# hsientzucheng/CP-360-Weakly-Supervised-Saliency

Hardware: AMD Instinct MI355X
Metric: frames/sec end-to-end 1024x2048 equi->saliency (higher is better)
Workload: dtype bf16+f16; 1 GPU; C3/C4 per-GPU shard: 4 clips x 16 frames 1024x2048 u8 equi -> 6x224^2 cube -> CubePad ResNet-50 -> CAM -> ConvLSTM x16 -> cube_to_equi saliency 14x28; clips_per_gpu=4, frames_per_clip=16, cube_dim=224, graph_replay=False, temporal_stage_dtype=bf16, static_stage_dtype=f16, static_stage_fp16_fallback=False, parallelism=clips sharded over 1 GPU(s), 1 all-gather of maps, pipelining=SaliencyEngine.stream: two HIP streams, fill + drain inside the timed region

## Files before the change

### cp_360_weakly_supervised_saliency_amd/csrc/conv_igemm.hip

```cpp
#include "common.h"
#include <stdio.h>
#include <stdlib.h>

#include "conv_common.h"

template <typename T, int MJ>
__device__ __forceinline__ void epilogue_direct(const ConvK& p, f32x4 (&acc)[4][MJ], int n0, int m0, int wch0, int wrow0,
                                                int lane, int rows_valid) {
    constexpr int JB = sizeof(T) == 4 ? 2 : 5;
    const int ml = lane & 15;
    const T* res = reinterpret_cast<const T*>(p.res);
    T* outp = reinterpret_cast<T*>(p.out);
    const int rlim = min(rows_valid, p.M - m0);
#pragma unroll
    for (int pr = 0; pr < 2; ++pr) {
        const int n = n0 + wch0 + pr * 32 + (lane >> 4) * 8;
        const bool nok = n < p.c_out;
        float bb[8] = {0.f, 0.f, 0.f, 0.f, 0.f, 0.f, 0.f, 0.f};
        if (p.bias && nok) {
            const float4 t0 = *reinterpret_cast<const float4*>(p.bias + n);
            const float4 t1 = *reinterpret_cast<const float4*>(p.bias + n + 4);
            bb[0] = t0.x; bb[1] = t0.y; bb[2] = t0.z; bb[3] = t0.w; bb[4] = t1.x; bb[5] = t1.y; bb[6] = t1.z; bb[7] = t1.w;
        }
#pragma unroll
// ... 765 lines not shown
#undef CP360_RING_TAIL
    }

    const int ml = lane & 15;
    if (!p.partial && p.epi_direct) {
        epilogue_direct<T, MJ>(p, acc, n0, m0, wch0, wrow0, lane, BM);
        return;
    }
    if (!p.partial && (p.c_out % EPC == 0) && (p.ld_out % EPC == 0) && (p.out_coff % EPC == 0) &&
        (p.ld_res % EPC == 0)) {
        epilogue_lds<T, BN, BM, MJ, 512, G::template lds_bytes<T>()>(p, lds, acc, n0, m0, wch0, wrow0, lane, tid);
        return;
    }
#pragma unroll
    for (int i = 0; i < 4; ++i) {
        const int n = n0 + wch0 + acc_chan(i, lane);
        if (n >= p.c_out) continue;
#pragma unroll
        for (int j = 0; j < MJ; ++j) {
            const int m = m0 + wrow0 + j * 16 + ml;
            if (m >= p.M) continue;
            float v[4] = {acc[i][j][0], acc[i][j][1], acc[i][j][2], acc[i][j][3]};
            if (p.partial) {
                store4(p.partial + ((size_t)split * p.M + m) * p.c_out + (p.slab_rows ? slab_col(n) : n), v);
            } else {
                if (p.bias) {
                    const float4 bb = *reinterpret_cast<const float4*>(p.bias + n);
                    v[0] += bb.x; v[1] += bb.y; v[2] += bb.z; v[3] += bb.w;
                }
                if (p.res) {
                    float r[4];
                    load4(reinterpret_cast<const T*>(p.res) + (size_t)m * p.ld_res + n, r);
                    v[0] += r[0]; v[1] += r[1]; v[2] += r[2]; v[3] += r[3];
                }
                if (p.relu) {
                    v[0] = fmaxf(v[0], 0.f); v[1] = fmaxf(v[1], 0.f);
                    v[2] = fmaxf(v[2], 0.f); v[3] = fmaxf(v[3], 0.f);
                }
                store4(reinterpret_cast<T*>(p.out) + (size_t)m * p.ld_out + p.out_coff + n, v);
            }
        }
    }
}

template <typename T, int BM>
__global__ __launch_bounds__(512, 2) void conv_igemm_ring_kernel(const ConvK p) {
    typedef RingGeom<BM> G;
    __shared__ __attribute__((aligned(1024))) unsigned char lds[G::template lds_bytes<T>()];

    const int tid = threadIdx.x, lane = tid & 63;
    const int wave = __builtin_amdgcn_readfirstlane(tid >> 6);
    int n0, m0, split;
    {
        const int nwg = p.nt * p.mt * p.splits;
        const int L = blockIdx.x, xcd = L & 7, q = nwg >> 3, r = nwg & 7;
        int w = (xcd < r ? xcd * (q + 1) : r * (q + 1) + (xcd - r) * q) + (L >> 3);
        if (p.reverse) w = nwg - 1 - w;
        int nt_i, mt_i;
        if (p.m_fast) {
            mt_i = w % p.mt;
            const int rest = w / p.mt;
            nt_i = rest % p.nt;
            split = rest / p.nt;
        } else {
            nt_i = w % p.nt;
            const int rest = w / p.nt;
            mt_i = rest % p.mt;
            split = rest / p.mt;
        }
        n0 = nt_i * G::BN;
        m0 = mt_i * BM;
    }
    if constexpr (BM == 256) {
        if (wave < 4) ring_body<T, 256, 8, 4, false>(p, lds, n0, m0, split, wave, lane, tid, (wave >> 1) * 64, (wave & 1) * 128);
        else          ring_body<T, 256, 8, 4, true>(p, lds, n0, m0, split, wave, lane, tid, (wave >> 1) * 64, (wave & 1) * 128);
    } else if constexpr (BM == 160) {
        if (wave < 4) ring_body<T, 160, 5, 3, false>(p, lds, n0, m0, split, wave, lane, tid, (wave >> 1) * 64, (wave & 1) * 80);
        else          ring_body<T, 160, 5, 3, true>(p, lds, n0, m0, split, wave, lane, tid, (wave >> 1) * 64, (wave & 1) * 80);
    } else {
        static_assert(BM == 304, "pixel tile is 160, 256 or 304");
        if (wave < 4) ring_body<T, 304, 10, 5, false>(p, lds, n0, m0, split, wave, lane, tid, wave * 64, 0);
        else          ring_body<T, 304, 9, 5, true>(p, lds, n0, m0, split, wave, lane, tid, (wave - 4) * 64, 160);
    }
}

template <typename T>
__global__ __launch_bounds__(512, 4) void conv_igemm_ring2_kernel(const ConvK p) {
    typedef RingGeom<128, 2> G;
    __shared__ __attribute__((aligned(1024))) unsigned char lds[G::template lds_bytes<T>()];
    const int tid = threadIdx.x, lane = tid & 63;
    const int wave = __builtin_amdgcn_readfirstlane(tid >> 6);
    int n0, m0, split;
    {
        const int nwg = p.nt * p.mt * p.splits;
        const int L = blockIdx.x, xcd = L & 7, q = nwg >> 3, r = nwg & 7;
        int w = (xcd < r ? xcd * (q + 1) : r * (q + 1) + (xcd - r) * q) + (L >> 3);
        if (p.reverse) w = nwg - 1 - w;
        int nt_i, mt_i;
        if (p.m_fast) {
            mt_i = w % p.mt;
            const int rest = w / p.mt;
            nt_i = rest % p.nt;
            split = rest / p.nt;
        } else {
            nt_i = w % p.nt;
            const int rest = w / p.nt;
            mt_i = rest % p.mt;
            split = rest / p.mt;
        }
        n0 = nt_i * G::BN;
        m0 = mt_i * 128;
    }
    if (wave < 4) ring_body<T, 128, 4, 2, false, 2>(p, lds, n0, m0, split, wave, lane, tid, (wave >> 1) * 64, (wave & 1) * 64);
    else          ring_body<T, 128, 4, 2, true, 2>(p, lds, n0, m0, split, wave, lane, tid, (wave >> 1) * 64, (wave & 1) * 64);
}

__device__ __forceinline__ int clip_swz(int row) { return ((row >> 2) & 1) << 1; }

template <int MODE> struct ClipGeom {
    static constexpr bool FACE = MODE == 1, HALF = MODE == 2;
    static constexpr int BN = 256, BM = FACE ? 256 : HALF ? 192 : 304, NW = 6, NA = 2;
    static constexpr int RROWS = FACE ? 336 : HALF ? 384 : 304;
    static constexpr int GROUP_ROWS = FACE ? 128 : HALF ? 96 : 160;
    static constexpr int XW = (RROWS - 256) / 16;
    static constexpr int WSTAGE = BN * 64;
    static constexpr int ATILE = RROWS * 64;
    static constexpr int TAB_ROW = 32;
    static constexpr int TAB_BYTES = 9 * 2 * 16 * TAB_ROW;
    static constexpr int OFF_ACT = NW * WSTAGE;
    static constexpr int OFF_TAB = OFF_ACT + NA * ATILE;
    static constexpr int LDS_BYTES = OFF_TAB + TAB_BYTES;
};

template <typename T, int MJ, int JH, bool LAG, int MODE>
__device__ __forceinline__ void clip_body(const ConvK& p, unsigned char* lds, const int n0, const int clip, const int split,
                                          const int wave, const int lane, const int tid, const int wch0, const int grp) {
    typedef ClipGeom<MODE> G;
    constexpr bool FACE = G::FACE, HALF = G::HALF;
    constexpr int BN = G::BN, BM = G::BM;
    constexpr int EPC = Elem<T>::EPC;
    constexpr int BKS = 4 * EPC;
    constexpr int TAPS = 9;
    const int wrow0 = grp * G::GROUP_ROWS;
    const bool xw = wave < G::XW;
    const int rows_valid = FACE ? 256 : HALF ? 192 : p.clip_rows;
    const int m0 = clip * rows_valid;

    const int drow = 16 * wave + (lane >> 2);
    const int dchunk = (lane & 3) ^ ((0 - ((4 * wave + (lane >> 4)) & 3)) & 3);
    const int dchunk_a = (lane & 3) ^ clip_swz(drow);
    const T* in = reinterpret_cast<const T*>(p.in);
    const T* wbase = reinterpret_cast<const T*>(p.w) + (size_t)(n0 / 256) * 256 * p.k_total + drow * BKS + dchunk * EPC;
    constexpr int wpass = 128 * BKS;
    constexpr int WSTEP = 256 * BKS;
    const unsigned lds_base = (unsigned)(size_t)lds;
    const unsigned lds_wave = lds_base + (unsigned)(16 * wave) * 64;
    int aoff[3];
#pragma unroll
    for (int q = 0; q < 3; ++q) {
        const int r = drow + 128 * q;
        int off = -1;
        if (FACE) {
            if (r < 18 * 18 && (q < 2 || xw)) {
                const int cube = clip / 6, f = clip - cube * 6;
                const CubePadGeom geom{16, 1, 1, 1, 1};
                off = (cube * 6 * 256 + cubepad_src(f, r / 18, r - (r / 18) * 18, geom)) * p.pix_stride;
// ... 388 lines not shown
__global__ __launch_bounds__(256) void pack_weights_kernel(const float* __restrict__ w, const float* __restrict__ scale,
                                                           T* __restrict__ packed, int c_out, int c_out_pad, int c_in,
                                                           int c_pad, int kh, int kw, int stem_mode, int chan_major,
                                                           const float* __restrict__ w2, const float* __restrict__ scale2,
                                                           int c_in2, int c_pad2) {
    const int taps = kh * kw;
    constexpr int BKS = 64 / (int)sizeof(T);
    const int ktot = taps * c_pad + c_pad2;
    const long long total = (long long)c_out_pad * ktot;
    for (long long idx = (long long)blockIdx.x * blockDim.x + threadIdx.x; idx < total;
         idx += (long long)gridDim.x * blockDim.x) {
        int c, tap, n;
        if (c_pad2 > 0) {
            const int k = (int)(idx % ktot);
            n = (int)(idx / ktot);
            tap = min(k / c_pad, taps);
            c = k - tap * c_pad;
        } else if (chan_major) {
            const int e = (int)(idx % BKS);
            long long t = idx / BKS;
            const int r = (int)(t % 256);
            t /= 256;
            tap = (int)(t % taps);
            t /= taps;
            const int cpb = c_pad / BKS;
            c = (int)(t % cpb) * BKS + e;
            n = (int)(t / cpb) * 256 + r;
        } else {
            c = (int)(idx % c_pad);
            const long long t = idx / c_pad;
            tap = (int)(t % taps);
            n = (int)(t / taps);
        }
        n = (n & ~31) + ((n >> 2) & 3) * 8 + ((n >> 4) & 1) * 4 + (n & 3);
        float v = 0.f;
        if (n < c_out && tap >= taps) {
            if (c < c_in2) v = w2[(size_t)n * c_in2 + c] * (scale2 ? scale2[n] : 1.f);
        } else if (n < c_out) {
            if (stem_mode) {
                const int kx = c >> 2, ch = c & 3, ky = tap;
                if (c < c_in && kx < 7 && ch < 3) v = w[(((size_t)n * 3 + ch) * 7 + ky) * 7 + kx];
            } else if (c < c_in) {
                const int ky = tap / kw, kx = tap - ky * kw;
                v = w[(((size_t)n * c_in + c) * kh + ky) * kw + kx];
            }
            if (scale) v *= scale[n];
        }
        if constexpr (sizeof(T) == 4)
            packed[idx] = v;
        else if constexpr (__is_same(T, f16_raw))
            packed[idx] = (f16_raw)v;
        else
            packed[idx] = f32_to_bf16(v);
    }
}

static int elem_bytes(int dtype) { return dtype == CP360_F32 ? 4 : ((dtype == CP360_BF16 || dtype == CP360_F16) ? 2 : 0); }
static int bk_of(int dtype) { return 128 / elem_bytes(dtype); }
static int c_pad_of(const cp360_conv_desc* d) {
    const int unit = d->clip_resident ? bk_of(d->dtype) / 2 : bk_of(d->dtype);
    return (d->c_in + unit - 1) / unit * unit;
}
static int round_up(int a, int b) { return (a + b - 1) / b * b; }
static int c_pad2_of(const cp360_conv_desc* d) { return d->c_in2 > 0 ? round_up(d->c_in2, bk_of(d->dtype)) : 0; }

static int small_shape_status(const cp360_conv_desc* d) {
    if (d->clip_resident || d->c_out % 8 != 0) return CP360_ERR_UNSUPPORTED;
    if (d->kh * d->kw + (d->c_in2 > 0 ? 1 : 0) > CP360_SMALL_MAX_TAPS) return CP360_ERR_UNSUPPORTED;
    const long long es = elem_bytes(d->dtype);
    if ((long long)d->n_img * d->h_in * d->w_in * d->pix_stride * es >= (1LL << 32)) return CP360_ERR_UNSUPPORTED;
    if (d->c_in2 > 0 && (long long)d->n_img * d->h_in2 * d->w_in2 * d->pix_stride2 * es >= (1LL << 32)) return CP360_ERR_UNSUPPORTED;
    if (64LL * ((long long)d->kh * d->kw * c_pad_of(d) + c_pad2_of(d)) * es >= (1LL << 32)) return CP360_ERR_UNSUPPORTED;
    if (d->dtype != CP360_F32 && (d->ld_out % 8 != 0 || d->out_coff % 8 != 0 || d->ld_res % 8 != 0)) return CP360_ERR_ALIGN;
    return CP360_OK;
}

static int check_desc(const cp360_conv_desc* d) {
    if (!d) return CP360_ERR_NULL;
    if (d->dtype != CP360_F32 && d->dtype != CP360_BF16 && d->dtype != CP360_F16) return CP360_ERR_BAD_DTYPE;
    if (d->n_img <= 0 || d->h_in <= 0 || d->w_in <= 0 || d->c_in <= 0 || d->kh <= 0 || d->kw <= 0 || d->sy <= 0 ||
        d->sx <= 0 || d->h_out <= 0 || d->w_out <= 0 || d->c_out <= 0 || d->splits < 1 || d->pix_stride <= 0)
        return CP360_ERR_BAD_SHAPE;
    const int epc = 16 / elem_bytes(d->dtype);
    if (d->tile_px != 0 && d->tile_px != 64 && d->tile_px != 128 && d->tile_px != 129 && d->tile_px != 160 && d->tile_px != 256 &&
        d->tile_px != 304 && d->tile_px != 6464)
        return CP360_ERR_BAD_SHAPE;
    if (d->tile_px == 160 && d->dtype == CP360_F32) return CP360_ERR_UNSUPPORTED;
    if (d->tile_px == 6464) {
        const int rc = small_shape_status(d);
        if (rc) return rc;
    }
    if (d->tile_px == 129 && d->dtype == CP360_F32) return CP360_ERR_UNSUPPORTED;
    if (d->slab_rows != 0 && d->slab_rows != 1) return CP360_ERR_BAD_SHAPE;
    if (d->slab_rows && d->c_out % 32 != 0) return CP360_ERR_ALIGN;
    if (d->clip_resident != 0 && d->clip_resident != 1) return CP360_ERR_BAD_SHAPE;
    if (d->clip_resident && !(d->pad_mode == 1 && d->pad == 1 && d->kh == 3 && d->kw == 3 && d->sy == 1 && d->sx == 1 &&
                              d->h_in == d->w_in && (6 * d->h_in * d->w_in <= 304 || d->h_in == 16 || d->h_in == 8) && d->c_out >= 256 &&
                              d->pix_stride >= d->c_in && d->tile_px == 0))
        return CP360_ERR_UNSUPPORTED;
    if (d->c_in2 < 0) return CP360_ERR_BAD_SHAPE;
    if (d->c_in2 > 0) {
        if (d->clip_resident || d->c_out < 256 || d->pix_stride < d->c_in) return CP360_ERR_UNSUPPORTED;
        if (d->c_in2 % epc != 0) return CP360_ERR_ALIGN;
        if (d->pix_stride2 < d->c_in2 || d->h_in2 <= 0 || d->w_in2 <= 0 || d->sy2 <= 0 || d->sx2 <= 0 ||
            (d->h_out - 1) * d->sy2 >= d->h_in2 || (d->w_out - 1) * d->sx2 >= d->w_in2)
            return CP360_ERR_BAD_SHAPE;
        if ((long long)d->n_img * d->h_in2 * d->w_in2 * d->pix_stride2 >= (1LL << 31)) return CP360_ERR_BAD_SHAPE;
    }
    if (d->c_in % epc != 0 || d->c_out % 4 != 0 || d->ld_out % 4 != 0 || d->out_coff % 4 != 0 || d->ld_res % 4 != 0)
        return CP360_ERR_ALIGN;
    if (d->ld_out < d->c_out + d->out_coff) return CP360_ERR_BAD_SHAPE;
    if (d->pad_mode) {
        if (d->n_img % 6 != 0) return CP360_ERR_BATCH_NOT_6N;
        if (d->h_in != d->w_in) return CP360_ERR_NOT_SQUARE;
        if (d->pad < 0 || d->pad > d->h_in) return CP360_ERR_BAD_SHAPE;
    }
    const int pad2 = d->pad_mode ? 2 * d->pad : 0;
    if ((d->h_out - 1) * d->sy + d->kh > d->h_in + pad2) return CP360_ERR_BAD_SHAPE;
    const int span = d->pix_stride >= d->c_in ? 1 : (d->c_in + d->pix_stride - 1) / d->pix_stride;
    if (span > 1 && d->pad_mode) return CP360_ERR_UNSUPPORTED;
    if ((d->w_out - 1) * d->sx + (d->kw - 1) + span > d->w_in + pad2) return CP360_ERR_BAD_SHAPE;
    if ((long long)d->n_img * d->h_in * d->w_in * d->pix_stride >= (1LL << 31)) return CP360_ERR_BAD_SHAPE;
    return CP360_OK;
}

extern "C" size_t cp360_conv_packed_bytes(const cp360_conv_desc* d) {
    if (check_desc(d)) return 0;
    return (size_t)round_up(d->c_out, 256) * ((size_t)d->kh * d->kw * c_pad_of(d) + c_pad2_of(d)) * elem_bytes(d->dtype);
}

extern "C" size_t cp360_conv_partial_bytes(const cp360_conv_desc* d) {
    if (check_desc(d) || d->splits <= 1) return 0;
    return (size_t)d->splits * d->n_img * d->h_out * d->w_out * d->c_out * sizeof(float);
}

struct ConvPlan {
    int bn, bm, slots, splits;
    double cost;
    long long wgs = 0;
};

static ConvPlan plan_candidate(const cp360_conv_desc* d, int bn, int bm, int slots, double t_step) {
    const long long M = (long long)d->n_img * d->h_out * d->w_out;
    const long long wgs = ((d->c_out + bn - 1) / bn) * ((M + bm - 1) / bm);
    const int bk = bk_of(d->dtype);
    const int nsteps = d->kh * d->kw * (round_up(d->c_in, bk) / bk) + c_pad2_of(d) / bk;
    if (d->dtype == CP360_F32) t_step *= 3.0;
    const double t_fixed = 4.0;
    ConvPlan best{bn, bm, slots, 1, 0.0};
    for (int s = 1; s <= 32; ++s) {
        if (s > 1 && nsteps / s < 8) break;
        const long long rounds = (wgs * s + slots - 1) / slots;
        const int steps = (nsteps + s - 1) / s;
        double cost = (double)rounds * (t_fixed + steps * t_step);
        if (s > 1) cost += 4.0 + (double)s * (double)M * d->c_out * 8.0 / 4.0e6;
        if (s == 1 || cost < best.cost) {
            best.splits = s;
            best.cost = cost;
            best.wgs = wgs * s;
        }
    }
    return best;
}

static bool small_eligible(const cp360_conv_desc* d) {
    return d->dtype == CP360_F32 && small_shape_status(d) == CP360_OK;
}

static ConvPlan plan_small(const cp360_conv_desc* d) {
    const long long M = (long long)d->n_img * d->h_out * d->w_out;
    const long long tiles = ((d->c_out + 63) / 64) * ((M + 63) / 64);
    const int bk = bk_of(d->dtype);
    const int nsteps = d->kh * d->kw * (round_up(d->c_in, bk) / bk) + c_pad2_of(d) / bk;
    const double t_step = d->dtype == CP360_F32 ? 0.7 : 0.35;
    ConvPlan best{64, 64, 1024, 1, 0.0};
    for (int s = 1; s <= 32; ++s) {
        if (s > 1 && nsteps / s < 4) break;
        const long long W = tiles * s;
        const int steps = (nsteps + s - 1) / s;
        const long long per_cu = d->dtype == CP360_F32 ? (W + 255) / 256 : (W + 1023) / 1024;
        double cost = (double)((W + 1023) / 1024) * 3.0 + (double)per_cu * steps * t_step;
        if (s > 1) cost += 4.0 + (double)s * (double)M * d->c_out * 8.0 / 4.0e6;
        if (s == 1 || cost < best.cost) {
            best.splits = s;
            best.cost = cost;
            best.wgs = W;
        }
    }
    return best;
}

static ConvPlan plan_big(const cp360_conv_desc* d);
static int clip_tiles(const cp360_conv_desc* d) { return d->h_in == 16 ? d->n_img : d->h_in == 8 ? d->n_img / 3 : d->n_img / 6; }

static ConvPlan plan_of(const cp360_conv_desc* d) {
    ConvPlan best = plan_big(d);
    if (d->tile_px == 6464) return plan_small(d);
    if (d->tile_px == 0 && small_eligible(d)) {
        const ConvPlan sm = plan_small(d);
        if (sm.cost < best.cost || best.wgs < 256) best = sm;
    }
    return best;
}

static ConvPlan plan_big(const cp360_conv_desc* d) {
    if (d->clip_resident) {
        const int wgs = ((d->c_out + 255) / 256) * clip_tiles(d);
        const int nsub = 9 * (c_pad_of(d) / (bk_of(d->dtype) / 2));
        const double t_sub = (d->dtype == CP360_F32 ? 2.7 : 0.9) * (d->h_in == 8 ? 0.7 : 1.0);
        const long long M = (long long)d->n_img * d->h_out * d->w_out;
        ConvPlan best{256, 304, 256, 1, 0.0};
        for (int s = 1; s <= 32; ++s) {
            if (s > 1 && nsub / s < 16) break;
            const int rounds = (wgs * s + 255) / 256;
            double cost = (double)rounds * (4.0 + (double)((nsub + s - 1) / s) * t_sub);
            if (s > 1) cost += 4.0 + (double)s * (double)M * d->c_out * 8.0 / 4.0e6;
            if (s == 1 || cost < best.cost) {
                best.splits = s;
                best.cost = cost;
                best.wgs = (long long)wgs * s;
            }
        }
        return best;
    }
    if (d->c_out <= 64) return plan_candidate(d, 64, 256, 512, 1.5);
    if (d->c_out < 256) return plan_candidate(d, 128, 128, 512, 1.5);
    ConvPlan best = plan_candidate(d, 256, 256, 256, 2.2);
    const ConvPlan b = plan_candidate(d, 256, 128, 256, 1.25);
    if (b.cost < best.cost) best = b;
    const ConvPlan c = plan_candidate(d, 256, 304, 256, 2.2 * 304.0 / 256.0);
    if (c.cost < best.cost) best = c;
    if (d->dtype != CP360_F32 && d->c_in2 == 0) {
        const ConvPlan t160 = plan_candidate(d, 256, 160, 256, 2.2 * 176.0 / 256.0);
        if (t160.cost < best.cost) best = t160;
    }
    const int kbytes = (d->c_in + d->c_in2) * elem_bytes(d->dtype);
    if (d->dtype != CP360_F32 && d->kh * d->kw == 1 && kbytes >= 256 && kbytes <= 512) {
        ConvPlan r2 = plan_candidate(d, 256, 128, 512, 1.25);
        r2.bm = 129;
        if (r2.cost < best.cost) best = r2;
    }
    if (d->c_in2 > 0 && best.bm == 128) best.bm = d->dtype == CP360_F32 ? 256 : 129;
    return best;
}

static void tile_of(const cp360_conv_desc* d, int* bn, int* bm, int* slots) {
    ConvPlan pl = plan_of(d);
    *bn = pl.bn;
    *bm = pl.bm;
    *slots = pl.slots;
    if (pl.bm == 64) return;
    if (d->c_out >= 256 && d->tile_px == 64) {
        *bn = 128;
        *bm = 128;
        *slots = 512;
    } else if (d->c_out >= 256 && d->tile_px) {
        *bn = 256;
        *bm = d->tile_px;
        *slots = 256;
    }
}

extern "C" int cp360_conv_suggest_splits(const cp360_conv_desc* d) {
    cp360_conv_desc t = *d;
    t.splits = 1;
    if (check_desc(&t)) return 1;
    return plan_of(&t).splits;
}

extern "C" int cp360_conv_prefer_clip(const cp360_conv_desc* d) {
    if (!d) return 0;
    cp360_conv_desc c = *d;
    c.splits = 1;
    c.tile_px = 0;
    c.clip_resident = 1;
    if (check_desc(&c)) return 0;
    cp360_conv_desc t = c;
    t.clip_resident = 0;
    if (check_desc(&t) || !small_eligible(&t)) return 1;
    return plan_big(&c).cost <= plan_small(&t).cost ? 1 : 0;
}

extern "C" int cp360_conv_plan_describe(const cp360_conv_desc* d, char* buf, size_t cap) {
    if (!d || !buf || cap == 0) return CP360_ERR_NULL;
    cp360_conv_desc t = *d;
    t.splits = 1;
    int rc = check_desc(&t);
    if (rc) return rc;
    const ConvPlan pl = plan_of(&t);
    int bn = 0, bm = 0, slots = 0;
    tile_of(&t, &bn, &bm, &slots);
    const long long M = (long long)t.n_img * t.h_out * t.w_out;
    const char* name;
    long long wgs;
    if (t.clip_resident) {
        name = t.h_in == 16 ? "conv_clip 256 ch x one 16x16 face (activations LDS-resident)"
               : t.h_in == 8 ? "conv_clip 256 ch x half a cube of 8x8 faces (the cube LDS-resident)"
                             : "conv_clip 256 ch x one cube (activations LDS-resident)";
        wgs = (long long)((t.c_out + 255) / 256) * clip_tiles(&t);
    } else if (bm == 64) {
        name = "conv_small 64 ch x 64 px (8 waves)";
        wgs = (long long)((t.c_out + 63) / 64) * ((M + 63) / 64);
    } else if (t.c_out < 256 || bn != 256) {
        const bool narrow = t.c_out <= 64;
        name = narrow ? "conv_igemm 64 ch x 256 px (4 waves)" : "conv_igemm 128 ch x 128 px (4 waves)";
        wgs = narrow ? (long long)((t.c_out + 63) / 64) * ((M + 255) / 256) : (long long)((t.c_out + 127) / 128) * ((M + 127) / 128);
    } else {
        const int px = bm == 129 ? 128 : bm;
        name = bm == 129 ? "conv_igemm_ring2 256 ch x 128 px (two workgroups per CU)"
               : bm == 304 ? "conv_igemm_ring 256 ch x 304 px" : bm == 160 ? "conv_igemm_ring 256 ch x 160 px" : bm >= 256 ? "conv_igemm_ring 256 ch x 256 px" : "conv_igemm_dma 256 ch x 128 px";
        wgs = (long long)((t.c_out + 255) / 256) * ((M + px - 1) / px);
    }
    const int n = snprintf(buf, cap, "%s, %lld workgroups x split-K %d%s, model %.0f us", name, wgs * pl.splits, pl.splits,
                           t.c_in2 > 0 ? " (+ second source)" : "", pl.cost);
    return n < 0 ? CP360_ERR_BAD_SHAPE : (n >= (int)cap ? (int)cap - 1 : n);
}

static int pack_weights_impl(const cp360_conv_desc* d, const float* w_oihw, const float* scale, const float* w2,
                             const float* scale2, void* packed, int stem_mode, void* stream);

extern "C" int cp360_conv_pack_weights(const cp360_conv_desc* d, const float* w_oihw, const float* scale, void* packed,
                                       int stem_mode, void* stream) {
    if (d && d->c_in2 > 0) return CP360_ERR_NULL;
    return pack_weights_impl(d, w_oihw, scale, nullptr, nullptr, packed, stem_mode, stream);
}

extern "C" int cp360_conv_pack_weights2(const cp360_conv_desc* d, const float* w_oihw, const float* scale,
                                        const float* w2_oi, const float* scale2, void* packed, void* stream) {
    if (!d || d->c_in2 <= 0) return CP360_ERR_BAD_SHAPE;
    if (!w2_oi) return CP360_ERR_NULL;
    return pack_weights_impl(d, w_oihw, scale, w2_oi, scale2, packed, 0, stream);
}

static int pack_weights_impl(const cp360_conv_desc* d, const float* w_oihw, const float* scale, const float* w2,
                             const float* scale2, void* packed, int stem_mode, void* stream) {
    int rc = check_desc(d);
    if (rc) return rc;
    if (!w_oihw || !packed) return CP360_ERR_NULL;
    if (stem_mode && !(d->kh == 7 && d->kw == 1 && d->c_in == 32)) return CP360_ERR_UNSUPPORTED;
    if (stem_mode && d->clip_resident) return CP360_ERR_UNSUPPORTED;
    const int c_pad = c_pad_of(d);
    const int c_out_pad = round_up(d->c_out, 256);
    const int c_pad2 = c_pad2_of(d);
    const long long total = (long long)c_out_pad * ((long long)d->kh * d->kw * c_pad + c_pad2);
    long long blocks = (total + 255) / 256;
    if (blocks > 4096) blocks = 4096;
    hipStream_t st = (hipStream_t)stream;
    if (d->dtype == CP360_F32)
        hipLaunchKernelGGL((pack_weights_kernel<float>), dim3((unsigned)blocks), dim3(256), 0, st, w_oihw, scale,
                           (float*)packed, d->c_out, c_out_pad, d->c_in, c_pad, d->kh, d->kw, stem_mode, d->clip_resident,
                           w2, scale2, d->c_in2, c_pad2);
    else if (d->dtype == CP360_F16)
        hipLaunchKernelGGL((pack_weights_kernel<f16_raw>), dim3((unsigned)blocks), dim3(256), 0, st, w_oihw, scale,
                           (f16_raw*)packed, d->c_out, c_out_pad, d->c_in, c_pad, d->kh, d->kw, stem_mode, d->clip_resident,
                           w2, scale2, d->c_in2, c_pad2);
    else
        hipLaunchKernelGGL((pack_weights_kernel<bf16_raw>), dim3((unsigned)blocks), dim3(256), 0, st, w_oihw, scale,
                           (bf16_raw*)packed, d->c_out, c_out_pad, d->c_in, c_pad, d->kh, d->kw, stem_mode, d->clip_resident,
                           w2, scale2, d->c_in2, c_pad2);
    CP360_CHECK_HIP();
    return CP360_OK;
}

template <typename T, int WN, int WM>
static void launch_conv(ConvK& k, hipStream_t st) {
    k.nt = (k.c_out + WN * 64 - 1) / (WN * 64);
    k.mt = (k.M + WM * 64 - 1) / (WM * 64);
    k.m_fast = ((long long)k.c_out * k.k_total > (long long)k.M * k.kh * k.kw * k.c_in) ? 1 : 0;
    dim3 grid((unsigned)(k.nt * k.mt * k.splits), 1, 1);
    hipLaunchKernelGGL((conv_igemm_kernel<T, WN, WM>), grid, dim3(256), 0, st, k);
}

template <typename T>
static int launch_wide(const ConvK& k, int bm, dim3 grid, hipStream_t st) {
    if (bm == 304) hipLaunchKernelGGL((conv_igemm_ring_kernel<T, 304>), grid, dim3(512), 0, st, k);
    else if (bm == 160) {
        if constexpr (sizeof(T) == 2) hipLaunchKernelGGL((conv_igemm_ring_kernel<T, 160>), grid, dim3(512), 0, st, k);
        else return CP360_ERR_UNSUPPORTED;
    } else if (bm >= 256) hipLaunchKernelGGL((conv_igemm_ring_kernel<T, 256>), grid, dim3(512), 0, st, k);
    else hipLaunchKernelGGL((conv_igemm_dma_kernel<T, 4>), grid, dim3(512), 0, st, k);
    return CP360_OK;
}

extern "C" int cp360_conv_forward(const cp360_conv_desc* d, const void* in, const void* packed_w, const float* bias,
                                  const void* residual, void* out, float* partial, void* stream) {
    return cp360_conv_forward2(d, in, nullptr, packed_w, bias, residual, out, partial, stream);
}

extern "C" int cp360_conv_forward2(const cp360_conv_desc* d, const void* in, const void* in2, const void* packed_w,
                                   const float* bias, const void* residual, void* out, float* partial, void* stream) {
    int rc = check_desc(d);
    if (rc) return rc;
    if (!in || !packed_w) return CP360_ERR_NULL;
    if ((d->c_in2 > 0) != (in2 != nullptr)) return CP360_ERR_NULL;
    if (d->splits > 1 && !partial) return CP360_ERR_NULL;
    if (d->splits == 1 && !out && !partial) return CP360_ERR_NULL;
    if (residual && d->ld_res < d->c_out) return CP360_ERR_BAD_SHAPE;
    ConvK k;
    k.in = (const unsigned char*)in;
    k.w = (const unsigned char*)packed_w;
    k.out = (unsigned char*)out;
    k.bias = bias;
    k.res = (const unsigned char*)residual;
    k.partial = (d->splits > 1 || !out) ? partial : nullptr;
    k.n_img = d->n_img; k.h_in = d->h_in; k.w_in = d->w_in; k.c_in = d->c_in; k.pix_stride = d->pix_stride;
    k.kh = d->kh; k.kw = d->kw; k.sy = d->sy; k.sx = d->sx; k.h_out = d->h_out; k.w_out = d->w_out;
    k.c_out = d->c_out; k.pad_mode = d->pad_mode; k.pad = d->pad; k.ld_out = d->ld_out; k.out_coff = d->out_coff;
    k.ld_res = d->ld_res; k.relu = d->relu; k.splits = d->splits;
    k.hw_out = d->h_out * d->w_out;
    k.M = d->n_img * k.hw_out;
    const int bk = bk_of(d->dtype);
    k.c_pad = c_pad_of(d);
    k.steps_per_tap = k.c_pad / bk;
    k.in2 = (const unsigned char*)in2;
    k.c_in2 = d->c_in2; k.c_pad2 = c_pad2_of(d); k.pix_stride2 = d->pix_stride2; k.h_in2 = d->h_in2; k.w_in2 = d->w_in2;
    k.sy2 = d->sy2; k.sx2 = d->sx2;
    k.ntap = d->kh * d->kw;
    k.nsteps = d->kh * d->kw * k.steps_per_tap + k.c_pad2 / bk;
    k.steps_per_split = (k.nsteps + d->splits - 1) / d->splits;
    k.k_total = d->kh * d->kw * k.c_pad + k.c_pad2;
    k.slab_rows = d->slab_rows;
    k.reverse = cp360_launch_reverse();
    k.clip_rows = 6 * d->h_out * d->w_out;
    k.nsub = k.k_total / (bk / 2);
    k.sub_per_split = (k.nsub + d->splits - 1) / d->splits;
    {
        const size_t wbytes = (size_t)((d->c_out + 255) / 256) * 256 * k.k_total * (d->dtype == CP360_F32 ? 4 : 2);
        k.w_pin = wbytes >= ((size_t)96 << 20) ? 8 : 0x7fffffff;
    }
    k.epi_direct = 0;
    hipStream_t st = (hipStream_t)stream;
    if (d->clip_resident) {
        const int mode = d->h_in == 16 ? 1 : d->h_in == 8 ? 2 : 0;
        k.nt = (k.c_out + 255) / 256;
        k.mt = clip_tiles(d);
        k.m_fast = 1;
        dim3 grid((unsigned)(k.nt * k.mt * k.splits), 1, 1);
#define CP360_CLIP(TT)                                                                                    \
        {                                                                                                     \
            if (mode == 1)      hipLaunchKernelGGL((conv_clip_kernel<TT, 1>), grid, dim3(512), 0, st, k);     \
            else if (mode == 2) hipLaunchKernelGGL((conv_clip_kernel<TT, 2>), grid, dim3(512), 0, st, k);     \
            else                hipLaunchKernelGGL((conv_clip_kernel<TT, 0>), grid, dim3(512), 0, st, k);     \
        }
        if (d->dtype == CP360_F32) CP360_CLIP(float)
        else if (d->dtype == CP360_F16) CP360_CLIP(f16_raw)
        else CP360_CLIP(bf16_raw)
#undef CP360_CLIP
        CP360_CHECK_HIP();
        return CP360_OK;
    }
    const bool narrow = d->c_out <= 64;
    int bn_ = 0, bm_ = 0, slots_ = 0;
    tile_of(d, &bn_, &bm_, &slots_);
    if (bm_ == 64) {
        cp360_launch_conv_small(k, d->dtype, st);
        CP360_CHECK_HIP();
        return CP360_OK;
    }
    if (d->dtype != CP360_F32 && d->kh == 1 && d->kw == 1 && d->sy == 1 && d->sx == 1 && d->pad == 0 && d->c_in == 64 &&
        d->c_out == 64 && d->c_in2 == 0 && d->splits <= 1 && !residual && d->tile_px == 0 && d->pix_stride % 8 == 0 &&
        d->ld_out % 8 == 0 && d->out_coff % 8 == 0 && k.M >= 4096 && k.out != nullptr && k.partial == nullptr) {
        long long blocks = ((long long)(k.M + 15) / 16 + 7) / 8;
        if (blocks > 256 * 8) blocks = 256 * 8;
        if (d->dtype == CP360_F16) hipLaunchKernelGGL((conv_pw64_kernel<f16_raw>), dim3((unsigned)blocks), dim3(256), 0, st, k);
        else hipLaunchKernelGGL((conv_pw64_kernel<bf16_raw>), dim3((unsigned)blocks), dim3(256), 0, st, k);
        CP360_CHECK_HIP();
        return CP360_OK;
    }
    if (d->c_out < 256) bn_ = bm_ = slots_ = 0;
    const bool wide = d->c_out >= 256 && bn_ == 256;
    if (d->c_in2 > 0) {
        if (!wide) return CP360_ERR_UNSUPPORTED;
        if (bm_ == 128) bm_ = d->dtype == CP360_F32 ? 256 : 129;
    }
    if (wide) {
        const bool big = bm_ >= 256;
        const int bm = bm_ == 129 ? 128 : bm_;
        if (bm_ == 129) k.epi_direct = d->c_out % 8 == 0 && d->ld_out % 8 == 0 && d->out_coff % 8 == 0 && d->ld_res % 8 == 0;
        k.nt = (k.c_out + 255) / 256;
        k.mt = (k.M + bm - 1) / bm;
        k.m_fast = ((long long)k.c_out * k.k_total > (long long)k.M * k.kh * k.kw * k.c_in) ? 1 : 0;
        dim3 grid((unsigned)(k.nt * k.mt * k.splits), 1, 1);
        if (d->c_in2 > 0 && !big && bm_ != 129) return CP360_ERR_UNSUPPORTED;
        if (bm_ == 129 && d->dtype == CP360_F16) hipLaunchKernelGGL((conv_igemm_ring2_kernel<f16_raw>), grid, dim3(512), 0, st, k);
        else if (bm_ == 129) hipLaunchKernelGGL((conv_igemm_ring2_kernel<bf16_raw>), grid, dim3(512), 0, st, k);
        else if (d->dtype == CP360_F32) rc = launch_wide<float>(k, bm, grid, st);
        else if (d->dtype == CP360_F16) rc = launch_wide<f16_raw>(k, bm, grid, st);
        else rc = launch_wide<bf16_raw>(k, bm, grid, st);
        if (rc) return rc;
    } else if (d->dtype == CP360_F32) {
        if (narrow) launch_conv<float, 1, 4>(k, st);
        else launch_conv<float, 2, 2>(k, st);
    } else if (d->dtype == CP360_F16) {
        if (narrow) launch_conv<f16_raw, 1, 4>(k, st);
        else launch_conv<f16_raw, 2, 2>(k, st);
    } else {
        if (narrow) launch_conv<bf16_raw, 1, 4>(k, st);
        else launch_conv<bf16_raw, 2, 2>(k, st);
    }
    CP360_CHECK_HIP();
    return CP360_OK;
}

extern "C" int cp360_conv_finish(const cp360_conv_desc* d, const float* partial, const float* bias,
                                 const void* residual, void* out, void* stream) {
    return cp360_conv_finish_add(d, partial, nullptr, bias, residual, out, stream);
}

extern "C" int cp360_conv_finish_add(const cp360_conv_desc* d, const float* partial, const float* extra, const float* bias,
                                     const void* residual, void* out, void* stream) {
    int rc = check_desc(d);
    if (rc) return rc;
    if (!partial || !out) return CP360_ERR_NULL;
    const int M = d->n_img * d->h_out * d->w_out;
    const long long total = (long long)M * (d->c_out / 4);
    long long blocks = (total + 255) / 256;
    if (blocks > 2048) blocks = 2048;
    hipStream_t st = (hipStream_t)stream;
    if (d->dtype == CP360_F32)
        hipLaunchKernelGGL((conv_finish_kernel<float>), dim3((unsigned)blocks), dim3(256), 0, st, partial, d->splits,
                           bias, (const float*)residual, d->ld_res, (float*)out, d->ld_out, d->out_coff, M, d->c_out,
                           d->relu, d->slab_rows, extra);
    else if (d->dtype == CP360_F16)
        hipLaunchKernelGGL((conv_finish_kernel<f16_raw>), dim3((unsigned)blocks), dim3(256), 0, st, partial,
                           d->splits, bias, (const f16_raw*)residual, d->ld_res, (f16_raw*)out, d->ld_out,
                           d->out_coff, M, d->c_out, d->relu, d->slab_rows, extra);
    else
        hipLaunchKernelGGL((conv_finish_kernel<bf16_raw>), dim3((unsigned)blocks), dim3(256), 0, st, partial,
                           d->splits, bias, (const bf16_raw*)residual, d->ld_res, (bf16_raw*)out, d->ld_out,
                           d->out_coff, M, d->c_out, d->relu, d->slab_rows, extra);
    CP360_CHECK_HIP();
    return CP360_OK;
}

extern "C" int cp360_lstm_gates(const float* gates_partial, int splits, const float* bias, const float* c_prev,
                                float* c_next, void* h_out, int h_dtype, int ld_h, int h_coff, float* h_f32, int M,
                                int Hc, int slab_rows, void* stream) {
    return cp360_lstm_gates_next(gates_partial, splits, bias, c_prev, c_next, h_out, h_dtype, ld_h, h_coff, h_f32, M, Hc,
                                 slab_rows, nullptr, nullptr, 0, 0, 0, stream);
}

extern "C" int cp360_lstm_gates_next(const float* gates_partial, int splits, const float* bias, const float* c_prev,
                                     float* c_next, void* h_out, int h_dtype, int ld_h, int h_coff, float* h_f32, int M,
                                     int Hc, int slab_rows, const float* x_next, const float* minmax, int x_coff,
                                     int P, size_t clip_stride, void* stream) {
    if (!gates_partial || !bias || !c_prev || !c_next || !h_out) return CP360_ERR_NULL;
    if (x_next && (!minmax || P <= 0 || M % P != 0 || x_coff % 4 != 0 || clip_stride % 4 != 0 || x_coff + Hc > ld_h ||
                   (x_coff < h_coff + Hc && h_coff < x_coff + Hc)))
        return CP360_ERR_BAD_SHAPE;
    if (splits < 1 || M <= 0 || Hc <= 0) return CP360_ERR_BAD_SHAPE;
    if (Hc % 4 != 0 || ld_h % 4 != 0 || h_coff % 4 != 0) return CP360_ERR_ALIGN;
    if (slab_rows && (4 * Hc) % 32 != 0) return CP360_ERR_ALIGN;
    const long long total = (long long)M * (Hc / 4);
    long long blocks = (total + 255) / 256;
    if (blocks > 2048) blocks = 2048;
    hipStream_t st = (hipStream_t)stream;
    if (h_dtype == CP360_F32)
        hipLaunchKernelGGL((lstm_gates_kernel<float>), dim3((unsigned)blocks), dim3(256), 0, st, gates_partial, splits,
                           bias, c_prev, c_next, (float*)h_out, ld_h, h_coff, h_f32, M, Hc, slab_rows, x_next, minmax, x_coff, P, clip_stride);
    else if (h_dtype == CP360_BF16)
        hipLaunchKernelGGL((lstm_gates_kernel<bf16_raw>), dim3((unsigned)blocks), dim3(256), 0, st, gates_partial,
                           splits, bias, c_prev, c_next, (bf16_raw*)h_out, ld_h, h_coff, h_f32, M, Hc, slab_rows, x_next, minmax, x_coff, P,
                           clip_stride);
    else if (h_dtype == CP360_F16)
        hipLaunchKernelGGL((lstm_gates_kernel<f16_raw>), dim3((unsigned)blocks), dim3(256), 0, st, gates_partial,
                           splits, bias, c_prev, c_next, (f16_raw*)h_out, ld_h, h_coff, h_f32, M, Hc, slab_rows, x_next, minmax, x_coff, P,
                           clip_stride);
    else
        return CP360_ERR_BAD_DTYPE;
    CP360_CHECK_HIP();
    return CP360_OK;
// ... 2 lines not shown
```

Baseline: 5358 frames/s.

## Add three-stage full-line ring conv kernel for 1x1 stride-1 16-bit convs

Adds a new implicit-GEMM kernel variant (256 channels x 160 pixels) that stages full 128-byte K lines with a three-deep LDS ring and a lag-split wave schedule, refilling one stage while computing on another. The planner selects it for 1x1 stride-1 unpadded 16-bit convolutions through a discounted cost estimate. The intent is to hide global-to-LDS latency better than the existing 160-pixel ring. In exchange it uses much more LDS per workgroup (two workgroups per CU) and relies on a heuristic cost factor.

Result: no change. 5356 frames/s (median of 6 runs) (-0.0%).

```diff
diff --git a/cp_360_weakly_supervised_saliency_amd/csrc/conv_igemm.hip b/cp_360_weakly_supervised_saliency_amd/csrc/conv_igemm.hip
--- a/cp_360_weakly_supervised_saliency_amd/csrc/conv_igemm.hip
+++ b/cp_360_weakly_supervised_saliency_amd/csrc/conv_igemm.hip
@@ -871,6 +871,232 @@
         if (wave < 4) ring_body<T, 304, 10, 5, false>(p, lds, n0, m0, split, wave, lane, tid, wave * 64, 0);
         else          ring_body<T, 304, 9, 5, true>(p, lds, n0, m0, split, wave, lane, tid, (wave - 4) * 64, 160);
     }
+}
+
+template <int BM> struct RingFlGeom {
+    static constexpr int BN = 256, NSTAGE = 3;
+    static constexpr int A_PASSES = BN / 64;
+    static constexpr int B_FULL = BM / 64, B_REM = BM % 64;
+    static constexpr int B_PASSES = B_FULL + (B_REM ? 1 : 0);
+    static constexpr int XWAVES = B_REM / 8;
+    static constexpr int DMA_BASE = A_PASSES + B_FULL;
+    static constexpr int STAGE = (BN + BM) * 128;
+    template <typename T> static constexpr int lds_bytes() {
+        return NSTAGE * STAGE > RingGeom<BM>::template epi_bytes<T>() ? NSTAGE * STAGE : RingGeom<BM>::template epi_bytes<T>();
+    }
+};
+
+template <typename T, int BM, int MJ, bool LAG>
+__device__ __forceinline__ void ringfl_body(const ConvK& p, unsigned char* lds, const int n0, const int m0, const int split,
+                                            const int wave, const int lane, const int tid, const int wch0,
+                                            const int wrow0) {
+    typedef RingFlGeom<BM> G;
+    constexpr int BN = G::BN, STAGE = G::STAGE, NS = G::NSTAGE, A_PASSES = G::A_PASSES, B_PASSES = G::B_PASSES;
+    constexpr int EPC = Elem<T>::EPC;
+    constexpr int BK = 8 * EPC;
+    constexpr int D0 = G::DMA_BASE, D1 = G::DMA_BASE + 1;
+    static_assert(sizeof(T) == 2, "the full-line ring is built for the 16-bit types");
+    static_assert(NS * STAGE <= 160 * 1024, "three stages must fit the CU's LDS");
+    const bool xw = G::XWAVES > 0 && wave < G::XWAVES;
+
+    const int drow = 8 * wave + (lane >> 3);
+    const int dchunk = (lane & 7) ^ ((4 * wave + (lane >> 4)) & 7);
+
+    int roff[B_PASSES];
+    const CubePadGeom geom{p.h_in, p.pad, p.pad, p.pad, p.pad};
+    auto set_tap = [&](int tap) __attribute__((always_inline)) {
+        const int ky = tap / p.kw, kx = tap - ky * p.kw;
+#pragma unroll
+        for (int pb = 0; pb < B_PASSES; ++pb) {
+            const int m = m0 + drow + 64 * pb;
+            int off = -1;
+            if (m < p.M && (pb < G::B_FULL || xw)) {
+                const int img = m / p.hw_out, rem = m - img * p.hw_out;
+                const int oy = rem / p.w_out, ox = rem - oy * p.w_out;
+                const int py = oy * p.sy + ky, px = ox * p.sx + kx;
+                int pix;
+                if (p.pad_mode) {
+                    const int grp = img / 6, f = img - grp * 6;
+                    pix = grp * 6 * p.h_in * p.w_in + cubepad_src(f, py, px, geom);
+                } else {
+                    pix = (img * p.h_in + py) * p.w_in + px;
+                }
+                off = pix * p.pix_stride;
+            }
+            roff[pb] = off;
+        }
+    };
+
+    const int s_begin = split * p.steps_per_split;
+    const int nloc = min(p.nsteps, s_begin + p.steps_per_split) - s_begin;
+    int tap = s_begin / p.steps_per_tap;
+    int c0 = (s_begin - tap * p.steps_per_tap) * BK;
+
+    const T* in = reinterpret_cast<const T*>(p.in);
+    const T* wbase = reinterpret_cast<const T*>(p.w) + (size_t)(n0 + drow) * p.k_total + dchunk * EPC;
+    const size_t wpass = (size_t)64 * p.k_total;
+    const unsigned lds_wave = (unsigned)(size_t)lds + (unsigned)(8 * wave) * 128;
+
+    auto issue_one = [&](int q, unsigned sbase) __attribute__((always_inline)) {
+        if (q < A_PASSES) {
+            glds16(wbase + q * wpass + ((size_t)tap * p.c_pad + c0), sbase + q * 64 * 128);
+        } else {
+            const int pb = q - A_PASSES;
+            const int e = c0 + dchunk * EPC;
+            const bool ok = e < p.c_in && roff[pb] >= 0;
+            const T* src = ok ? in + (size_t)roff[pb] + e : reinterpret_cast<const T*>(g_zero16);
+            glds16(src, sbase + BN * 128 + pb * 64 * 128);
+        }
+    };
+    auto issue = [&](int stage) __attribute__((always_inline)) {
+        const unsigned sbase = __builtin_amdgcn_readfirstlane(lds_wave + (unsigned)stage * STAGE);
+#pragma unroll
+        for (int q = 0; q < D0; ++q) issue_one(q, sbase);
+        if (G::XWAVES > 0 && xw) issue_one(D0, sbase);
+    };
+    auto advance = [&]() __attribute__((always_inline)) {
+        c0 += BK;
+        if (c0 >= p.c_pad) {
+            c0 = 0;
+            ++tap;
+            set_tap(tap);
+        }
+    };
+
+    f32x4 acc[4][MJ];
+#pragma unroll
+    for (int i = 0; i < 4; ++i)
+#pragma unroll
+        for (int j = 0; j < MJ; ++j) acc[i][j] = f32x4{0.f, 0.f, 0.f, 0.f};
+
+    if (nloc > 0) {
+        const int lrow = lane & 15, lchunk = lane >> 4;
+        set_tap(tap);
+        issue(0);
+        if (nloc > 1) { advance(); issue(1); }
+        int stage = 0;
+        u32x4 a[4], b[MJ];
+        if (LAG) {
+#pragma unroll
+            for (int i = 0; i < 4; ++i) a[i] = u32x4{0u, 0u, 0u, 0u};
+#pragma unroll
+            for (int j = 0; j < MJ; ++j) b[j] = u32x4{0u, 0u, 0u, 0u};
+        }
+#define CP360_RINGFL_HEAD(KK, REFILL)                                                                      \
+        {                                                                                                  \
+            const unsigned char* As = lds + stage * STAGE;                                                 \
+            const unsigned char* Bs = As + BN * 128;                                                       \
+            _Pragma("unroll") for (int i = 0; i < 4; ++i)                                                  \
+                a[i] = *reinterpret_cast<const u32x4*>(As + lds_swz(wch0 + i * 16 + lrow, (KK) * 4 + lchunk)); \
+            _Pragma("unroll") for (int j = 0; j < MJ; ++j)                                                 \
+                b[j] = *reinterpret_cast<const u32x4*>(Bs + lds_swz(wrow0 + j * 16 + lrow, (KK) * 4 + lchunk)); \
+            if (REFILL) {                                                                                  \
+                advance();                                                                                 \
+                const unsigned sbase = __builtin_amdgcn_readfirstlane(lds_wave + (unsigned)(stage == 0 ? NS - 1 : stage - 1) * STAGE); \
+                _Pragma("unroll") for (int q = 0; q < D0; ++q) issue_one(q, sbase);                        \
+                if (G::XWAVES > 0 && xw) issue_one(D0, sbase);                                             \
+            }                                                                                              \
+            if ((KK) == 1) stage = stage == NS - 1 ? 0 : stage + 1;                                        \
+        }
+#define CP360_RINGFL_TAIL()                                                                                \
+        {                                                                                                  \
+            _Pragma("unroll") for (int j = 0; j < MJ; ++j)                                                 \
+                _Pragma("unroll") for (int i = 0; i < 4; ++i) mma_chunk<T>(acc[i][j], a[i], b[j]);         \
+        }
+#define CP360_RINGFL_SUB(KK, REFILL)                                                                       \
+        {                                                                                                  \
+            if (LAG) asm volatile("s_waitcnt lgkmcnt(0)" ::: "memory");                                    \
+            __builtin_amdgcn_s_barrier();                                                                  \
+            __builtin_amdgcn_sched_barrier(0);                                                             \
+            if (!LAG) CP360_RINGFL_HEAD(KK, REFILL) else CP360_RINGFL_TAIL()                               \
+            __builtin_amdgcn_sched_barrier(0);                                                             \
+            __builtin_amdgcn_s_barrier();                                                                  \
+            __builtin_amdgcn_sched_barrier(0);                                                             \
+            if (!LAG) CP360_RINGFL_TAIL() else CP360_RINGFL_HEAD(KK, REFILL)                               \
+        }
+        int it = 0;
+        for (; it + NS - 1 < nloc; ++it) {
+            if (xw) wait_vmcnt<D1>(); else wait_vmcnt<D0>();
+            CP360_RINGFL_SUB(0, true)
+            CP360_RINGFL_SUB(1, false)
+        }
+        for (; it < nloc; ++it) {
+            wait_vmcnt_upto<D1>(min(1, nloc - 1 - it) * (xw ? D1 : D0));
+            CP360_RINGFL_SUB(0, false)
+            CP360_RINGFL_SUB(1, false)
+        }
+        if (LAG) CP360_RINGFL_TAIL()
+#undef CP360_RINGFL_SUB
+#undef CP360_RINGFL_HEAD
+#undef CP360_RINGFL_TAIL
+    }
+
+    if (!p.partial && (p.c_out % EPC == 0) && (p.ld_out % EPC == 0) && (p.out_coff % EPC == 0) && (p.ld_res % EPC == 0)) {
+        epilogue_lds<T, BN, BM, MJ, 512, G::template lds_bytes<T>()>(p, lds, acc, n0, m0, wch0, wrow0, lane, tid);
+        return;
+    }
+    const int ml = lane & 15;
+#pragma unroll
+    for (int i = 0; i < 4; ++i) {
+        const int n = n0 + wch0 + acc_chan(i, lane);
+        if (n >= p.c_out) continue;
+#pragma unroll
+        for (int j = 0; j < MJ; ++j) {
+            const int m = m0 + wrow0 + j * 16 + ml;
+            if (m >= p.M) continue;
+            float v[4] = {acc[i][j][0], acc[i][j][1], acc[i][j][2], acc[i][j][3]};
+            if (p.partial) {
+                store4(p.partial + ((size_t)split * p.M + m) * p.c_out + (p.slab_rows ? slab_col(n) : n), v);
+            } else {
+                if (p.bias) {
+                    const float4 bb = *reinterpret_cast<const float4*>(p.bias + n);
+                    v[0] += bb.x; v[1] += bb.y; v[2] += bb.z; v[3] += bb.w;
+                }
+                if (p.res) {
+                    float r[4];
+                    load4(reinterpret_cast<const T*>(p.res) + (size_t)m * p.ld_res + n, r);
+                    v[0] += r[0]; v[1] += r[1]; v[2] += r[2]; v[3] += r[3];
+                }
+                if (p.relu) {
+                    v[0] = fmaxf(v[0], 0.f); v[1] = fmaxf(v[1], 0.f);
+                    v[2] = fmaxf(v[2], 0.f); v[3] = fmaxf(v[3], 0.f);
+                }
+                store4(reinterpret_cast<T*>(p.out) + (size_t)m * p.ld_out + p.out_coff + n, v);
+            }
+        }
+    }
+}
+
+template <typename T>
+__global__ __launch_bounds__(512, 2) void conv_igemm_ringfl_kernel(const ConvK p) {
+    typedef RingFlGeom<160> G;
+    __shared__ __attribute__((aligned(1024))) unsigned char lds[G::template lds_bytes<T>()];
+
+    const int tid = threadIdx.x, lane = tid & 63;
+    const int wave = __builtin_amdgcn_readfirstlane(tid >> 6);
+    int n0, m0, split;
+    {
+        const int nwg = p.nt * p.mt * p.splits;
+        const int L = blockIdx.x, xcd = L & 7, q = nwg >> 3, r = nwg & 7;
+        int w = (xcd < r ? xcd * (q + 1) : r * (q + 1) + (xcd - r) * q) + (L >> 3);
+        if (p.reverse) w = nwg - 1 - w;
+        int nt_i, mt_i;
+        if (p.m_fast) {
+            mt_i = w % p.mt;
+            const int rest = w / p.mt;
+            nt_i = rest % p.nt;
+            split = rest / p.nt;
+        } else {
+            nt_i = w % p.nt;
+            const int rest = w / p.nt;
+            mt_i = rest % p.mt;
+            split = rest / p.mt;
+        }
+        n0 = nt_i * G::BN;
+        m0 = mt_i * 160;
+    }
+    if (wave < 4) ringfl_body<T, 160, 5, false>(p, lds, n0, m0, split, wave, lane, tid, (wave >> 1) * 64, (wave & 1) * 80);
+    else          ringfl_body<T, 160, 5, true>(p, lds, n0, m0, split, wave, lane, tid, (wave >> 1) * 64, (wave & 1) * 80);
 }
 
 template <typename T>
@@ -1425,10 +1651,11 @@
         d->sx <= 0 || d->h_out <= 0 || d->w_out <= 0 || d->c_out <= 0 || d->splits < 1 || d->pix_stride <= 0)
         return CP360_ERR_BAD_SHAPE;
     const int epc = 16 / elem_bytes(d->dtype);
-    if (d->tile_px != 0 && d->tile_px != 64 && d->tile_px != 128 && d->tile_px != 129 && d->tile_px != 160 && d->tile_px != 256 &&
+    if (d->tile_px != 0 && d->tile_px != 64 && d->tile_px != 128 && d->tile_px != 129 && d->tile_px != 160 && d->tile_px != 161 && d->tile_px != 256 &&
         d->tile_px != 304 && d->tile_px != 6464)
         return CP360_ERR_BAD_SHAPE;
     if (d->tile_px == 160 && d->dtype == CP360_F32) return CP360_ERR_UNSUPPORTED;
+    if (d->tile_px == 161 && (d->dtype == CP360_F32 || d->c_in2 > 0 || d->c_out < 256)) return CP360_ERR_UNSUPPORTED;
     if (d->tile_px == 6464) {
         const int rc = small_shape_status(d);
         if (rc) return rc;
@@ -1576,6 +1803,11 @@
     if (d->dtype != CP360_F32 && d->c_in2 == 0) {
         const ConvPlan t160 = plan_candidate(d, 256, 160, 256, 2.2 * 176.0 / 256.0);
         if (t160.cost < best.cost) best = t160;
+        if (d->kh == 1 && d->kw == 1 && d->sy == 1 && d->sx == 1 && d->pad == 0 && d->pix_stride >= d->c_in) {
+            ConvPlan fl = plan_candidate(d, 256, 160, 256, 2.2 * 176.0 / 256.0 * 0.84);
+            fl.bm = 161;
+            if (fl.cost < best.cost) best = fl;
+        }
     }
     const int kbytes = (d->c_in + d->c_in2) * elem_bytes(d->dtype);
     if (d->dtype != CP360_F32 && d->kh * d->kw == 1 && kbytes >= 256 && kbytes <= 512) {
@@ -1649,8 +1881,9 @@
         name = narrow ? "conv_igemm 64 ch x 256 px (4 waves)" : "conv_igemm 128 ch x 128 px (4 waves)";
         wgs = narrow ? (long long)((t.c_out + 63) / 64) * ((M + 255) / 256) : (long long)((t.c_out + 127) / 128) * ((M + 127) / 128);
     } else {
-        const int px = bm == 129 ? 128 : bm;
+        const int px = bm == 129 ? 128 : bm == 161 ? 160 : bm;
         name = bm == 129 ? "conv_igemm_ring2 256 ch x 128 px (two workgroups per CU)"
+               : bm == 161 ? "conv_igemm_ringfl 256 ch x 160 px (full 128-byte lines, 3 stages)"
                : bm == 304 ? "conv_igemm_ring 256 ch x 304 px" : bm == 160 ? "conv_igemm_ring 256 ch x 160 px" : bm >= 256 ? "conv_igemm_ring 256 ch x 256 px" : "conv_igemm_dma 256 ch x 128 px";
         wgs = (long long)((t.c_out + 255) / 256) * ((M + px - 1) / px);
     }
@@ -1716,7 +1949,10 @@
 
 template <typename T>
 static int launch_wide(const ConvK& k, int bm, dim3 grid, hipStream_t st) {
-    if (bm == 304) hipLaunchKernelGGL((conv_igemm_ring_kernel<T, 304>), grid, dim3(512), 0, st, k);
+    if (bm == 161) {
+        if constexpr (sizeof(T) == 2) hipLaunchKernelGGL((conv_igemm_ringfl_kernel<T>), grid, dim3(512), 0, st, k);
+        else return CP360_ERR_UNSUPPORTED;
+    } else if (bm == 304) hipLaunchKernelGGL((conv_igemm_ring_kernel<T, 304>), grid, dim3(512), 0, st, k);
     else if (bm == 160) {
         if constexpr (sizeof(T) == 2) hipLaunchKernelGGL((conv_igemm_ring_kernel<T, 160>), grid, dim3(512), 0, st, k);
         else return CP360_ERR_UNSUPPORTED;
@@ -1818,7 +2054,7 @@
     }
     if (wide) {
         const bool big = bm_ >= 256;
-        const int bm = bm_ == 129 ? 128 : bm_;
+        const int bm = bm_ == 129 ? 128 : bm_ == 161 ? 160 : bm_;
         if (bm_ == 129) k.epi_direct = d->c_out % 8 == 0 && d->ld_out % 8 == 0 && d->out_coff % 8 == 0 && d->ld_res % 8 == 0;
         k.nt = (k.c_out + 255) / 256;
         k.mt = (k.M + bm - 1) / bm;
@@ -1827,9 +2063,9 @@
         if (d->c_in2 > 0 && !big && bm_ != 129) return CP360_ERR_UNSUPPORTED;
         if (bm_ == 129 && d->dtype == CP360_F16) hipLaunchKernelGGL((conv_igemm_ring2_kernel<f16_raw>), grid, dim3(512), 0, st, k);
         else if (bm_ == 129) hipLaunchKernelGGL((conv_igemm_ring2_kernel<bf16_raw>), grid, dim3(512), 0, st, k);
-        else if (d->dtype == CP360_F32) rc = launch_wide<float>(k, bm, grid, st);
-        else if (d->dtype == CP360_F16) rc = launch_wide<f16_raw>(k, bm, grid, st);
-        else rc = launch_wide<bf16_raw>(k, bm, grid, st);
+        else if (d->dtype == CP360_F32) rc = launch_wide<float>(k, bm_, grid, st);
+        else if (d->dtype == CP360_F16) rc = launch_wide<f16_raw>(k, bm_, grid, st);
+        else rc = launch_wide<bf16_raw>(k, bm_, grid, st);
         if (rc) return rc;
     } else if (d->dtype == CP360_F32) {
         if (narrow) launch_conv<float, 1, 4>(k, st);
```
